# CMU-Quake/hercules

Hardware: AMD Instinct MI355X
Metric: element-updates/sec (whole node) + achieved HBM GB/s, 64M-elem box (higher is better)
Workload: dtype f64

## Files before the change

### hercules_amd/capi.py

```python
import ctypes
import os

import numpy as np

_HERE = os.path.dirname(os.path.abspath(__file__))
_LIBPATH = os.environ.get("HQ_SOLVER_LIB") or os.path.join(_HERE, "csrc", "libhq_solver.so")

HQ_VARIANT_AUTO, HQ_VARIANT_SCATTER, HQ_VARIANT_PATCH = 0, 1, 2
IPC_BLOB_BYTES = 4096

EXPORTS = ["hq_device_count", "hq_last_error", "hq_create", "hq_destroy", "hq_get_info", "hq_get_info_sized", "hq_abi_version", "hq_comm_init_ipc_n",
           "hq_options_init", "hq_create_opts", "hq_get_options", "hq_real_bytes",
           "hq_comm_unique_id", "hq_comm_init", "hq_comm_selftest", "hq_group_link", "hq_group_run", "hq_set_source", "hq_run", "hq_sync", "hq_gather", "hq_gather3",
           "hq_download", "hq_upload", "hq_phase_force", "hq_phase_update", "hq_download_force",
           "hq_run_timed", "hq_dominant_kernel", "hq_plan_check", "hq_stencil_plan_check", "hq_check_finite",
           "hq_stencil_coefficients", "hq_brick_plan_check", "hq_brick_plan_check_n", "hq_comm_init_host",
           "hq_comm_ipc_export", "hq_comm_init_ipc", "hq_comm_init_loopback"]


class HqError(RuntimeError):
    pass


HOST_EXCHANGE_FN = ctypes.CFUNCTYPE(ctypes.c_int, ctypes.c_void_p, ctypes.c_int32, ctypes.POINTER(ctypes.c_int32),
                                    ctypes.POINTER(ctypes.c_int64), ctypes.POINTER(ctypes.c_void_p), ctypes.c_int32,
                                    ctypes.POINTER(ctypes.c_int32), ctypes.POINTER(ctypes.c_int64),
                                    ctypes.POINTER(ctypes.c_void_p), ctypes.c_int32)


class _Messenger(ctypes.Structure):
    _fields_ = [("procid", ctypes.c_int32), ("nodecount", ctypes.c_int32),
                ("mapping", ctypes.c_void_p)]


class _Schedule(ctypes.Structure):
    _fields_ = [("c_count", ctypes.c_int32), ("first_c", ctypes.POINTER(_Messenger)),
                ("s_count", ctypes.c_int32), ("first_s", ctypes.POINTER(_Messenger))]


# ... 18 lines not shown
                ("ragged_patches", ctypes.c_int32), ("brick_units", ctypes.c_int32),
                ("brick_nodes", ctypes.c_int64), ("brick_units_pernode", ctypes.c_int32),
                ("brick_units_het", ctypes.c_int32), ("pcie_h2d_bytes", ctypes.c_int64),
                ("pcie_d2h_bytes", ctypes.c_int64), ("transport", ctypes.c_int32), ("ipc_arena_coarse", ctypes.c_int32),
                ("ipc_arena_kind", ctypes.c_int32), ("debug_halo", ctypes.c_int32),
                ("brick_units_packed", ctypes.c_int32), ("brick_units_ragged", ctypes.c_int32),
                ("brick_stream", ctypes.c_int32), ("brick_units_ragged_het", ctypes.c_int32), ("timed_steps", ctypes.c_int64),
                ("t_step_us", ctypes.c_double), ("t_shell_us", ctypes.c_double), ("t_interior_us", ctypes.c_double),
                ("t_chain_us", ctypes.c_double), ("t_chain_exposed_us", ctypes.c_double)]


OPTION_FIELDS = ["no_bricks", "brick_cz", "brick_minz", "brick_minnodes", "brick_no_het", "brick_no_ntsame", "brick_by_component",
                 "brick_stream", "brick_no_faces", "brick_half_tiles", "brick_no_pack", "patch_pipe", "patch_threads", "patch_pmax", "patch_pmerge", "patch_psplit", "patch_nlmax",
                 "patch_vmax", "patch_ragged", "patch_no_lattice", "patch_no_stencil", "patch_no_uniform", "patch_no_iso",
                 "patch_no_ntsame", "patch_no_dedup", "patch_wform", "patch_merge_rounds", "overlap", "no_overlap", "reserve_cus",
                 "cu_mask", "no_fused_share", "group_copies", "debug_halo", "ipc_arena"]


class Options(ctypes.Structure):
    _fields_ = ([("size", ctypes.c_uint64)] + [(n, ctypes.c_int32) for n in OPTION_FIELDS] +
                [("ipc_timeout_ms", ctypes.c_double), ("loopback_delay_us", ctypes.c_double),
                 ("verbose", ctypes.c_int32), ("quiet", ctypes.c_int32),
                 ("brick_ragged", ctypes.c_int32), ("brick_ragged_minfill", ctypes.c_int32),
                 ("allow_env", ctypes.c_int32), ("brick_ragged_het", ctypes.c_int32), ("reserved0", ctypes.c_int32),
                 ("phase_timing", ctypes.c_int32)])

    def __init__(self, **kw):
        super().__init__()
        load_library().hq_options_init(ctypes.byref(self), ctypes.c_uint64(ctypes.sizeof(self)))
        for k, v in kw.items():
            if k not in dict(self._fields_):
                raise TypeError("hq_options has no field %r" % k)
            setattr(self, k, v)

    def as_dict(self):
        return {k: getattr(self, k) for k, _ in self._fields_ if k != "size"}


_lib = None
_lib_f32 = None
_LIBPATH_F32 = os.environ.get("HQ_SOLVER_LIB_F32") or os.path.join(_HERE, "csrc", "libhq_solver_f32.so")


def load_library(path=None, precision="f64"):
    global _lib, _lib_f32
    if precision == "f32" and path is None:
        if _lib_f32 is None:
# ... 229 lines not shown
    _check(load_library().hq_plan_check(ctypes.byref(desc), rep))
    return dict(zip(PLAN_REPORT, [int(v) for v in rep]))


STENCIL_PLAN_REPORT = ("patches", "tables", "full_lattices", "boundary_nodes", "corners_checked", "faults")


def stencil_plan_check(desc):
    rep = (ctypes.c_int64 * 6)()
    _check(load_library().hq_stencil_plan_check(ctypes.byref(desc), rep))
    return dict(zip(STENCIL_PLAN_REPORT, [int(v) for v in rep]))


BRICK_PLAN_REPORT = ("brick_nodes", "columns", "units", "units_one_nt_row", "het_units", "neighbours_checked",
                     "patch_nodes", "faults", "ragged_units", "ragged_nodes", "ragged_het_units", "ragged_het_nodes")


def brick_plan_check(desc):
    rep = (ctypes.c_int64 * len(BRICK_PLAN_REPORT))()
    _check(load_library().hq_brick_plan_check_n(ctypes.byref(desc), rep, ctypes.c_int32(len(BRICK_PLAN_REPORT))))
    return dict(zip(BRICK_PLAN_REPORT, [int(v) for v in rep]))


def comm_unique_id():
    buf = (ctypes.c_char * 128)()
    _check(load_library().hq_comm_unique_id(buf))
    return bytes(buf)


def group_link(solvers):
    arr = (ctypes.c_void_p * len(solvers))(*[s._h for s in solvers])
    lib = solvers[0]._lib
    _check(lib.hq_group_link(arr, ctypes.c_int32(len(solvers))), lib)


def group_run(solvers, nsteps):
    arr = (ctypes.c_void_p * len(solvers))(*[s._h for s in solvers])
    lib = solvers[0]._lib
    _check(lib.hq_group_run(arr, ctypes.c_int32(len(solvers)), ctypes.c_int32(nsteps)), lib)
    for s in solvers:
        s.sync()
```

### hercules_amd/csrc/hq_brick.h

```cpp
#ifndef HQ_BRICK_H
#define HQ_BRICK_H

#include <chrono>
#include <map>

#include "hq_patch.h"

#define HQ_BK_TX 64
#ifndef HQ_BK_TY
#define HQ_BK_TY 8
#endif
#define HQ_BK_THREADS (HQ_BK_TX * HQ_BK_TY)
#define HQ_BK_PY (HQ_BK_TX + 2)
#define HQ_BK_PLANE ((HQ_BK_TX + 2) * (HQ_BK_TY + 2))
#ifndef HQ_BK_ATTR
#define HQ_BK_ATTR
#endif
#define HQ_BK_NTSAME 1
#define HQ_BK_HET 2
#define HQ_BK_TOPFACE 8
#define HQ_BK_BOTFACE 16
#define HQ_BK_RAGGED 32
#define HQ_BK_PACKED 4
#ifndef HQ_BH_WAVES
#define HQ_BH_WAVES 8
#endif
#define HQ_BH_THREADS (64 * HQ_BH_WAVES)
#define HQ_BH_NRT (64 + 2 * (HQ_BH_WAVES - 1))
#define HQ_BH_TX 62
#define HQ_BH_TY (HQ_BH_WAVES - 1)
#define HQ_BH_PY 65
#define HQ_BH_CS HQ_BH_THREADS
#define HQ_BH_ROWS (65 * (HQ_BH_WAVES + 1))

struct hq_brick_unit {
    int64_t base;
    int64_t tab;
    int32_t nx, ny, np, flags;
    double  c1, c2, beta;
    double  m0, m2, m1;
    double  ft[7], fb[7];
    int64_t coef;
};

struct hq_brick_cfg {
    int cz = 32;
    int minz = 4;
    int minnodes = 512;
    int ragged = 1;
    int minfill = 128;
    int ragged_het = 1;
};

static hq_brick_cfg hq_brick_cfg_of(const hq_options& o)
{
    hq_brick_cfg c;
    c.cz = std::max(2, hq_value_or(o.brick_cz, c.cz));
    c.minz = std::max(1, hq_value_or(o.brick_minz, c.minz));
    c.minnodes = std::max(1, hq_value_or(o.brick_minnodes, c.minnodes));
    c.ragged = hq_value_or(o.brick_ragged, c.ragged) != 0;
    c.minfill = std::min(HQ_BK_THREADS, std::max(1, hq_value_or(o.brick_ragged_minfill, c.minfill)));
    c.ragged_het = hq_value_or(o.brick_ragged_het, c.ragged_het) != 0;
    return c;
}

struct hq_brick_host {
// ... 672 lines not shown
        a.insert(a.end(), b.begin(), b.end());
        a.insert(a.end(), h.begin(), h.end());
        a.insert(a.end(), hp.begin(), hp.end());
        a.insert(a.end(), rh.begin(), rh.end());
        a.insert(a.end(), rhp.begin(), rhp.end());
        B->units.swap(a);
        if (B->npacked + B->nrpacked == 0) { std::vector<float>().swap(B->coef32); std::vector<double>().swap(B->nt2); }
        if (verbose) fprintf(stderr, "  brick plan: %d units: %d with one n_t row of which %d ragged, %d per-element coefficients of which %d packed, %d ragged per-element of which %d packed\n",
                             (int)B->units.size(), B->nsame, B->nrag, B->nhet, B->npacked, B->nrhet, B->nrpacked);
        if (verbose && B->nrag) {
            int64_t pos = 0, own = 0, other = 0;
            for (const hq_brick_unit& U : B->units) {
                if (!(U.flags & HQ_BK_RAGGED)) continue;
                const int32_t* pl = B->tab.data() + U.tab + (int64_t)(U.np + 2) * (2 * (U.nx + 2) + 2 * U.ny);
                for (int64_t i = 0; i < (int64_t)U.nx * U.ny * (U.np + 2); i++) { pos++; own += pl[i] >= 0; other += pl[i] <= -2; }
            }
            fprintf(stderr, "  brick plan: ragged units: %lld positions, %lld owned, %lld loaded for their neighbours' sake\n", (long long)pos, (long long)own, (long long)other);
        }
    }
    return 0;
}


static __device__ __forceinline__ double hq_uniform(double v)
{
    const int lo = __builtin_amdgcn_readfirstlane(__double2loint(v)), hi = __builtin_amdgcn_readfirstlane(__double2hiint(v));
    return __hiloint2double(hi, lo);
}

template <bool PERNODE, bool BYCOMP, bool RAGGED = false>
__global__ void HQ_BK_ATTR __launch_bounds__(HQ_BK_THREADS, 4)
hq_k_brick(int32_t count, int32_t per_xcd, const hq_brick_unit* __restrict__ units, const int32_t* __restrict__ tab,
           const hq_real* __restrict__ u1g, const hq_real* __restrict__ u2g, hq_real* __restrict__ ung,
           const double* __restrict__ nt3, const int32_t* __restrict__ src_ptr, const int32_t* __restrict__ src_ent,
           const double* __restrict__ F, double dt2, hq_stencil_coef sc)
{
    __shared__ __align__(16) double s_w[2 * 3 * HQ_BK_PLANE];
    const int slot = (int)(blockIdx.x & 7) * per_xcd + (int)(blockIdx.x >> 3);
    if (slot >= count) return;
    const hq_brick_unit U = units[slot];
    const int nx = U.nx, ny = U.ny, np = U.np, nxy = nx * ny, nr = 2 * (nx + 2) + 2 * ny;
    const int t = threadIdx.x, lx = t & (HQ_BK_TX - 1), ly = t >> 6;
    const bool active = lx < nx && ly < ny;
    const int sidx = active ? ly * nx + lx : 0;
    const int myrow = (ly + 1) * HQ_BK_PY + lx + 1;
    const bool ring = t < nr;
    int rrow;
    {
        int rx, ry;
        if (t < nx + 2) { rx = t - 1; ry = -1; }
        else if (t < 2 * (nx + 2)) { rx = t - (nx + 2) - 1; ry = ny; }
        else if (t < 2 * (nx + 2) + ny) { rx = -1; ry = t - 2 * (nx + 2); }
        else { rx = nx; ry = t - 2 * (nx + 2) - ny; }
        rrow = (ry + 1) * HQ_BK_PY + rx + 1;
    }
    const int32_t* __restrict__ utab = tab + U.tab;
    const int rofs = ring ? t : 0;
    const int32_t* __restrict__ cap = utab + (int64_t)(np + 2) * nr;
    int32_t vOut = -1, vMid = RAGGED ? cap[sidx] : 0, vCur = RAGGED ? cap[nxy + sidx] : 0, vNext = 0;
    const int32_t id_lo = RAGGED ? (vMid >= 0 ? vMid : -vMid - 2) : cap[sidx];
    const double beta = U.beta;
    double P[6], Q[2];
// ... 157 lines not shown
    }
#undef HQ_BK_LOAD
#undef HQ_BK_PUT
}


#define HQ_BH_LDS (8 * (2 * 2 * 3 * HQ_BH_ROWS + 6 * HQ_BH_THREADS))
#ifndef HQ_BH_ABL
#define HQ_BH_ABL 0
#endif

static __device__ __forceinline__ double hq_dpp_from_next_lane(double v)
{
    int lo = __double2loint(v), hi = __double2hiint(v);
    lo = __builtin_amdgcn_update_dpp(0, lo, 0x130, 0xf, 0xf, true);
    hi = __builtin_amdgcn_update_dpp(0, hi, 0x130, 0xf, 0xf, true);
    return __hiloint2double(hi, lo);
}

static __device__ __forceinline__ int64_t hq_rag_node(int32_t v) { return v >= 0 ? (int64_t)v : (v <= -2 ? (int64_t)(-v - 2) : (int64_t)0); }

template <bool PACKED, bool RAGGED = false>
__global__ void __launch_bounds__(HQ_BH_THREADS, HQ_BH_WAVES == 12 ? 3 : 4)
hq_k_brick_het(int32_t count, int32_t per_xcd, const hq_brick_unit* __restrict__ units, const int32_t* __restrict__ tab,
               const void* __restrict__ coef_any, const hq_real* __restrict__ u1g, const hq_real* __restrict__ u2g,
               hq_real* __restrict__ ung, const double* __restrict__ nt3, const int32_t* __restrict__ src_ptr,
               const int32_t* __restrict__ src_ent, const double* __restrict__ F, double dt2, hq_mat_const mat)
{
    extern __shared__ __align__(16) double s_het[];
    hq_lds_double* const img = (hq_lds_double*)s_het;
    hq_lds_double* const xch = img + 2 * 2 * 3 * HQ_BH_ROWS;
    const int slot = (int)(blockIdx.x & 7) * per_xcd + (int)(blockIdx.x >> 3);
    if (slot >= count) return;
    const hq_brick_unit U = units[slot];
    const int nx = U.nx, ny = U.ny, np = U.np, nxy = nx * ny, nr = 2 * (nx + 2) + 2 * ny;
    const int t = threadIdx.x, lx = t & 63, ly = t >> 6;
    const bool owner = lx < nx && ly < ny;
    const int sidx = owner ? ly * nx + lx : 0;
    const int myrow = (ly + 1) * HQ_BH_PY + lx + 1;
    const int row0 = ly * HQ_BH_PY + lx;
    const int rq = ly == HQ_BH_WAVES - 1 ? lx : (lx >= 62 ? 64 + 2 * ly + (lx - 62) : -1);
    const bool ringA = rq >= 0 && rq < nr, ringB = rq >= 0 && rq + HQ_BH_NRT < nr;
    auto ring_row = [&](int r) {
        int rx, ry;
        if (r < nx + 2) { rx = r - 1; ry = -1; }
        else if (r < 2 * (nx + 2)) { rx = r - (nx + 2) - 1; ry = ny; }
        else if (r < 2 * (nx + 2) + ny) { rx = -1; ry = r - 2 * (nx + 2); }
        else { rx = nx; ry = r - 2 * (nx + 2) - ny; }
        return (ry + 1) * HQ_BH_PY + rx + 1;
    };
    const int rrowA = ringA ? ring_row(rq) : 0, rrowB = ringB ? ring_row(rq + HQ_BH_NRT) : 0;
    const int32_t* __restrict__ rtabA = tab + U.tab + (ringA ? rq : 0);
    const int32_t* __restrict__ rtabB = tab + U.tab + (ringB ? rq + HQ_BH_NRT : 0);
    const int32_t* __restrict__ cap = tab + U.tab + (int64_t)(np + 2) * nr;
    const int64_t id_lo = RAGGED ? 0 : cap[sidx], id_hi = RAGGED ? 0 : cap[nxy + sidx];
    int32_t vload = RAGGED ? cap[sidx] : 0, vnext = RAGGED ? cap[nxy + sidx] : 0, idA = -1, idB = -1;
// ... 210 lines not shown
        rec.push_back({ P->h_slot[k], (int32_t)(loaded[i] - P->h_first[k]), i });
    }
    if (rec.empty()) return 0;
    std::sort(rec.begin(), rec.end());
    std::vector<int32_t> ptr((size_t)P->nunits + 1, 0), ent(rec.size() * 2);
    for (auto& r : rec) ptr[(size_t)r[0] + 1]++;
    for (int32_t u = 0; u < P->nunits; u++) ptr[(size_t)u + 1] += ptr[(size_t)u];
    for (size_t k = 0; k < rec.size(); k++) { ent[2 * k] = rec[k][1]; ent[2 * k + 1] = rec[k][2]; }
    if (hipMalloc((void**)&P->d_src_ptr, 4 * ptr.size()) != hipSuccess) { P->d_src_ptr = nullptr; return -2; }
    if (hipMalloc((void**)&P->d_src_ent, 4 * ent.size()) != hipSuccess) {
        hipFree(P->d_src_ptr); P->d_src_ptr = nullptr; P->d_src_ent = nullptr;
        return -2;
    }
    if (hipMemcpy(P->d_src_ptr, ptr.data(), 4 * ptr.size(), hipMemcpyHostToDevice) != hipSuccess ||
        hipMemcpy(P->d_src_ent, ent.data(), 4 * ent.size(), hipMemcpyHostToDevice) != hipSuccess) {
        hipFree(P->d_src_ptr); hipFree(P->d_src_ent); P->d_src_ptr = nullptr; P->d_src_ent = nullptr;
        return -3;
    }
    *bytes += (int64_t)(4 * ptr.size() + 4 * ent.size());
    return 0;
}

static void hq_brick_launch(const hq_brick_plan* P, const hq_real* u1, const hq_real* u2, hq_real* un, const double* nt3,
                            const double* F, double dt2, hipStream_t stream, bool light = false)
{
    const int32_t cnt[7] = { P->nsame - P->nrag, P->nunits - P->nsame - P->nhet - P->nrhet, P->nhet - P->npacked, P->npacked, P->nrag,
                             P->nrhet - P->nrpacked, P->nrpacked };
    int32_t first = 0;
    for (int k4 = 0; k4 < 7; k4++) {
        const int k = k4 == 0 ? 0 : (k4 == 1 ? 4 : (k4 < 5 ? k4 - 1 : k4));
        const int32_t count = cnt[k];
        if (count <= 0) continue;
        const int per_xcd = (count + 7) / 8;
        const int32_t* sp = P->d_src_ptr ? P->d_src_ptr + first : nullptr;
#define HQ_BK_ARGS count, per_xcd, P->d_units + first, P->d_tab, u1, u2, un, nt3, sp, P->d_src_ent, (sp ? F : nullptr), dt2, hq_stencil().c
#ifdef HQ_EXPERIMENT
        const unsigned xpad = getenv("HQ_X_BRICK_LDS_PAD") ? (unsigned)atoi(getenv("HQ_X_BRICK_LDS_PAD")) : 0u;
        if (xpad && k == 0) {
            static bool once = false;
            if (!once) {
                once = true;
                hipFuncSetAttribute((const void*)hq_k_brick<false, true>, hipFuncAttributeMaxDynamicSharedMemorySize, (int)xpad);
                hipFuncSetAttribute((const void*)hq_k_brick<false, false>, hipFuncAttributeMaxDynamicSharedMemorySize, (int)xpad);
            }
            if (light) hq_k_brick<false, true><<<per_xcd * 8, HQ_BK_THREADS, xpad, stream>>>(HQ_BK_ARGS);
            else hq_k_brick<false, false><<<per_xcd * 8, HQ_BK_THREADS, xpad, stream>>>(HQ_BK_ARGS);
        } else
#endif
        if (k == 0 && light) hq_k_brick<false, true><<<per_xcd * 8, HQ_BK_THREADS, 0, stream>>>(HQ_BK_ARGS);
        else if (k == 0) hq_k_brick<false, false><<<per_xcd * 8, HQ_BK_THREADS, 0, stream>>>(HQ_BK_ARGS);
        else if (k == 1 && light) hq_k_brick<true, true><<<per_xcd * 8, HQ_BK_THREADS, 0, stream>>>(HQ_BK_ARGS);
        else if (k == 1) hq_k_brick<true, false><<<per_xcd * 8, HQ_BK_THREADS, 0, stream>>>(HQ_BK_ARGS);
        else if (k == 4 && light) hq_k_brick<false, true, true><<<per_xcd * 8, HQ_BK_THREADS, 0, stream>>>(HQ_BK_ARGS);
        else if (k == 4) hq_k_brick<false, false, true><<<per_xcd * 8, HQ_BK_THREADS, 0, stream>>>(HQ_BK_ARGS);
        else if (k == 2) hq_k_brick_het<false><<<per_xcd * 8, HQ_BH_THREADS, HQ_BH_LDS, stream>>>(count, per_xcd, P->d_units + first, P->d_tab, P->d_coef, u1, u2, un, nt3, sp,
                                                                                               P->d_src_ent, (sp ? F : nullptr), dt2, P->mat);
        else if (k == 3) hq_k_brick_het<true><<<per_xcd * 8, HQ_BH_THREADS, HQ_BH_LDS, stream>>>(count, per_xcd, P->d_units + first, P->d_tab, P->d_coef32, u1, u2, un, P->d_nt2, sp,
                                                                                   P->d_src_ent, (sp ? F : nullptr), dt2, P->mat);
        else if (k == 5) hq_k_brick_het<false, true><<<per_xcd * 8, HQ_BH_THREADS, HQ_BH_LDS, stream>>>(count, per_xcd, P->d_units + first, P->d_tab, P->d_coef, u1, u2, un, nt3, sp,
                                                                                                     P->d_src_ent, (sp ? F : nullptr), dt2, P->mat);
        else hq_k_brick_het<true, true><<<per_xcd * 8, HQ_BH_THREADS, HQ_BH_LDS, stream>>>(count, per_xcd, P->d_units + first, P->d_tab, P->d_coef32, u1, u2, un, P->d_nt2, sp,
                                                                                          P->d_src_ent, (sp ? F : nullptr), dt2, P->mat);
#undef HQ_BK_ARGS
        first += count;
    }
}

#endif
```

### hercules_amd/csrc/hq_engine.hip

```cpp
#include <hip/hip_runtime.h>
#include <dlfcn.h>
#include <stdint.h>
#include <stdio.h>
#include <stdlib.h>
#include <string.h>
#include <unistd.h>

#include <algorithm>
#include <chrono>
#include <vector>

#define HQ_SOLVER_IMPLEMENTATION 1
#include "../../include/hq_solver.h"
#include "hq_kernels.h"
#include "hq_opts.h"
#include "hq_patch.h"
#include "hq_brick.h"


static thread_local char g_err[512] = "";

static int hq_fail(int code, const char* fmt, const char* a = "", const char* b = "")
{
    snprintf(g_err, sizeof g_err, fmt, a, b);
// ... 139 lines not shown
    bool overlap = false;
    bool stream_masked = false;
    bool can_overlap = false;
    int reserve_cus = 8;
    int32_t nI = 0, nOI = 0;
    double* d_iforce = nullptr;
    int32_t* d_oi_node = nullptr;
    int32_t* d_oi_slot = nullptr;
    int32_t* d_oi_ptr = nullptr;
    int32_t* d_oi_pos = nullptr;
    int32_t* d_oi_fc = nullptr;
    int32_t  nSD = 0;
    int32_t* d_sd_dst = nullptr;
    int32_t* d_sd_ptr = nullptr;
    int32_t* d_sd_src = nullptr;
    int32_t* d_sd_deps = nullptr;
    hq_patch_plan plan;
    hq_brick_plan bricks;
    std::vector<int32_t> perm;
    bool debug_halo = false;
    unsigned long long dbg_send_epoch[4] = { 0, 0, 0, 0 }, dbg_recv_epoch[4] = { 0, 0, 0, 0 };
    int64_t* d_gkey = nullptr;
    int32_t* d_halo_err = nullptr;
    enum { HQ_CLK_STEP0 = 0, HQ_CLK_SHELL1, HQ_CLK_INT0, HQ_CLK_INT1, HQ_CLK_CHAIN0, HQ_CLK_CHAIN1, HQ_CLK_N, HQ_CLK_SLOTS = 64 };
    struct hq_clock_slot { hipEvent_t e[HQ_CLK_N] = {}; bool used[HQ_CLK_N] = {}; bool pending = false; };
    bool clock_skip = false;
    std::vector<hq_clock_slot> clock;
    size_t clock_at = 0;
    double clk_us[5] = { 0, 0, 0, 0, 0 };
    int64_t clk_steps = 0;
    std::vector<hipEvent_t> ev;
    hipEvent_t ev_span[2] = { nullptr, nullptr };
    bool timing = false;
    size_t ev_used = 0;
};

template <typename T>
static int hq_dev_alloc(hq_ctx* c, T** p, size_t count)
{
    size_t bytes = sizeof(T) * (count ? count : 1);
    hipError_t e = hipMalloc((void**)p, bytes);
    if (e != hipSuccess) return hq_fail(HQ_ERR_NOMEM, "hipMalloc(%s) failed: %s", "", hipGetErrorString(e));
    c->bytes += (int64_t)bytes;
    return HQ_OK;
}

#define HQ_TRY(x) do { int r_ = (x); if (r_ != HQ_OK) return r_; } while (0)
// ... 535 lines not shown
    if (c->cstream) {
        hipError_t e2 = hipStreamSynchronize(c->cstream);
        if (e == hipSuccess) e = e2;
    }
    if (c->bstream) {
        hipError_t e2 = hipStreamSynchronize(c->bstream);
        if (e == hipSuccess) e = e2;
    }
    return e;
}

static void hq_clock_harvest(hq_ctx* c, hq_ctx::hq_clock_slot& sl, bool wait)
{
    if (!sl.pending) return;
    for (int k = 0; k < hq_ctx::HQ_CLK_N; k++)
        if (sl.used[k] && (wait ? hipEventSynchronize(sl.e[k]) : hipEventQuery(sl.e[k])) != hipSuccess) return;
    auto span = [&](int a, int b, double* us) {
        float ms = 0;
        if (!sl.used[a] || !sl.used[b] || hipEventElapsedTime(&ms, sl.e[a], sl.e[b]) != hipSuccess) return false;
        *us = 1e3 * (double)ms;
        return true;
    };
    double shell = 0, interior = 0, chain = 0, t_int_end = 0, t_chain_end = 0, t_shell_end = 0;
    span(hq_ctx::HQ_CLK_STEP0, hq_ctx::HQ_CLK_SHELL1, &shell);
    span(hq_ctx::HQ_CLK_INT0, hq_ctx::HQ_CLK_INT1, &interior);
    span(hq_ctx::HQ_CLK_CHAIN0, hq_ctx::HQ_CLK_CHAIN1, &chain);
    span(hq_ctx::HQ_CLK_STEP0, hq_ctx::HQ_CLK_SHELL1, &t_shell_end);
    span(hq_ctx::HQ_CLK_STEP0, hq_ctx::HQ_CLK_INT1, &t_int_end);
    span(hq_ctx::HQ_CLK_STEP0, hq_ctx::HQ_CLK_CHAIN1, &t_chain_end);
    const double compute_end = std::max(t_shell_end, t_int_end);
    c->clk_us[0] += std::max(compute_end, t_chain_end);
    c->clk_us[1] += shell;
    c->clk_us[2] += interior;
    c->clk_us[3] += chain;
    c->clk_us[4] += std::max(0.0, t_chain_end - compute_end);
    c->clk_steps++;
    sl.pending = false;
    for (int k = 0; k < hq_ctx::HQ_CLK_N; k++) sl.used[k] = false;
}

static void hq_clock_harvest_all(hq_ctx* c, bool wait)
{
    for (auto& sl : c->clock) hq_clock_harvest(c, sl, wait);
}

static bool hq_clock_on(const hq_ctx* c) { return hq_set(c->opts.phase_timing) || c->timing; }

// ... 149 lines not shown
        if (hipStreamCreateWithPriority(&c->bstream, hipStreamNonBlocking, prio) != hipSuccess) { c->bstream = nullptr; return false; }
        if (hipEventCreateWithFlags(&c->ev_patches, hipEventDisableTiming) != hipSuccess ||
            hipEventCreateWithFlags(&c->ev_bricks, hipEventDisableTiming) != hipSuccess) return false;
        hipEventRecord(c->ev_patches, c->stream);
        hipEventRecord(c->ev_bricks, c->stream);
    }
    return true;
}

static int hq_phase(hq_ctx* c, int ph)
{
    const bool patch = (c->variant == HQ_VARIANT_PATCH);
    double* ftab = patch ? c->d_iforce : c->d_force;
    hq_real* unew = patch ? c->d_u[c->spare] : c->d_u[c->prev];
    switch (ph) {
    case 0:
        if (patch) {
            int32_t k = c->step - c->src_step0;
            const double* F = (c->nloaded > 0 && k >= 0 && k < c->src_nsteps)
                                  ? c->d_F + (int64_t)k * c->nloaded * 3 : nullptr;
            int32_t nb = c->plan.nb, ne = c->plan.ne;
            if (c->overlap && !hq_patch_uses_pers(&c->plan) && nb > 0 && nb + ne <= 2 * hq_value_or(c->opts.patch_merge_rounds, 2) * c->plan.grid_cus) { nb += ne; ne = 0; }
            const bool bs = hq_use_brick_stream(c);
            if (c->overlap) HQ_HIP(hipStreamWaitEvent(c->stream, c->ev_shared, 0));
            if (bs) {
                HQ_HIP(hipStreamWaitEvent(c->stream, c->ev_bricks, 0));
                if (c->ev_shared) HQ_HIP(hipStreamWaitEvent(c->bstream, c->ev_shared, 0));
                HQ_HIP(hipStreamWaitEvent(c->bstream, c->ev_patches, 0));
            }
            auto launch_bricks = [&]() {
                if (c->bricks.nunits > 0)
                    hq_brick_launch(&c->bricks, c->d_u[c->now], c->d_u[c->prev], c->d_u[c->spare], c->plan.d_nt3, F, c->dt2,
                                    bs ? c->bstream : c->stream, hq_given(c->opts.brick_by_component) ? c->opts.brick_by_component != 0 : c->overlap);
                if (bs) hipEventRecord(c->ev_bricks, c->bstream);
            };
            hq_mark(c);
            hq_clock_begin(c);
            hq_clock(c, hq_ctx::HQ_CLK_STEP0, c->stream);
            if (bs) hq_clock(c, hq_ctx::HQ_CLK_INT0, c->bstream);
            bool chain_marked = false;
            auto chain_released = [&]() {
                if (!chain_marked && c->overlap) hq_clock(c, hq_ctx::HQ_CLK_CHAIN0, c->cstream);
                chain_marked = true;
            };
            if (c->plan.ns > 0 || c->plan.nr > 0) {
                const int32_t head = c->overlap ? nb : nb + ne;
                hq_patch_launch(&c->plan, 0, head, c->d_u[c->now], c->d_u[c->prev], c->d_u[c->spare], c->d_nt, F, c->dt2,
                                c->d_iforce, c->stream);
                hq_patch_launch_stencil(&c->plan, 0, c->d_u[c->now], c->d_u[c->prev], c->d_u[c->spare], c->d_nt, F, c->dt2,
                                        c->d_iforce, c->stream);
                if (c->overlap) {
                    HQ_HIP(hipEventRecord(c->ev_bnd, c->stream));
                    HQ_HIP(hipStreamWaitEvent(c->cstream, c->ev_bnd, 0));
                    chain_released();
                    hq_patch_launch(&c->plan, nb, ne, c->d_u[c->now], c->d_u[c->prev], c->d_u[c->spare], c->d_nt, F, c->dt2,
                                    c->d_iforce, c->stream, c->reserve_cus);
                }
                hq_patch_launch_stencil(&c->plan, 1, c->d_u[c->now], c->d_u[c->prev], c->d_u[c->spare], c->d_nt, F, c->dt2,
                                        c->d_iforce, c->stream);
            } else {
                if (c->overlap) {
                    hq_patch_launch(&c->plan, 0, nb, c->d_u[c->now], c->d_u[c->prev], c->d_u[c->spare], c->d_nt, F, c->dt2,
                                    c->d_iforce, c->stream);
                    HQ_HIP(hipEventRecord(c->ev_bnd, c->stream));
                    HQ_HIP(hipStreamWaitEvent(c->cstream, c->ev_bnd, 0));
                    chain_released();
                    hq_patch_launch(&c->plan, nb, ne, c->d_u[c->now], c->d_u[c->prev], c->d_u[c->spare], c->d_nt, F,
                                    c->dt2, c->d_iforce, c->stream, c->reserve_cus);
                } else {
                    hq_patch_launch(&c->plan, 0, nb + ne, c->d_u[c->now], c->d_u[c->prev], c->d_u[c->spare], c->d_nt, F,
                                    c->dt2, c->d_iforce, c->stream);
                }
            }
            if (bs) HQ_HIP(hipEventRecord(c->ev_patches, c->stream));
            hq_clock(c, hq_ctx::HQ_CLK_SHELL1, c->stream);
            if (!bs) hq_clock(c, hq_ctx::HQ_CLK_INT0, c->stream);
            launch_bricks();
            hq_clock(c, hq_ctx::HQ_CLK_INT1, bs ? c->bstream : c->stream);
            if (!c->overlap && hq_has_transport(c)) hq_clock(c, hq_ctx::HQ_CLK_CHAIN0, c->stream);
            hq_mark(c);
        } else {
            HQ_TRY(hq_launch_source(c));
            HQ_TRY(hq_launch_element_scatter(c));
        }
        return HQ_OK;
    case 1: return hq_xchg_send(c, &c->dn, ftab, true, true);
    case 2:
        HQ_TRY(hq_xchg_recv(c, &c->dn, ftab, true, true));
        if (patch) {
            if (c->nSD)
                hq_k_distribute<<<hq_blocks(c->nSD * 3, 256), 256, 0, c->overlap ? c->cstream : c->stream>>>(
                    c->nSD, c->d_sd_dst, c->d_sd_ptr, c->d_sd_src, c->d_sd_deps, c->d_iforce);
        } else if (c->nSD) {
            hq_k_distribute<<<hq_blocks(c->nSD * 3, 256), 256, 0, c->stream>>>(
                c->nSD, c->d_sd_dst, c->d_sd_ptr, c->d_sd_src, c->d_sd_deps, c->d_force);
        }
        return HQ_OK;
    case 3: return hq_xchg_send(c, &c->an, ftab, true, true);
    case 4:
        if (patch) {
            hipStream_t xs = c->overlap ? c->cstream : c->stream;
// ... 1063 lines not shown
    g_brick_check_extra[1] = 0;
    g_brick_check_extra[2] = B.nrhet;
    g_brick_check_extra[3] = 0;
    for (const hq_brick_unit& U : B.units) {
        if (!(U.flags & HQ_BK_RAGGED)) continue;
        const int32_t* pl = B.tab.data() + U.tab + (int64_t)(U.np + 2) * (2 * (U.nx + 2) + 2 * U.ny);
        for (int64_t i = (int64_t)U.nx * U.ny; i < (int64_t)U.nx * U.ny * (U.np + 1); i++) g_brick_check_extra[(U.flags & HQ_BK_HET) ? 3 : 1] += pl[i] >= 0;
    }
    if (bad) return hq_fail(HQ_ERR_STATE, "brick plan self-check failed%s", "");
    return HQ_OK;
}

extern "C" int hq_brick_plan_check_n(const hq_desc* d, int64_t* report, int32_t n)
{
    int64_t r8[8] = { 0, 0, 0, 0, 0, 0, 0, 0 };
    if (!report || n < 8) return hq_fail(HQ_ERR_ARG, "hq_brick_plan_check_n: a report of at least 8 entries%s", "");
    for (int k = 0; k < 4; k++) g_brick_check_extra[k] = 0;
    const int rc = hq_brick_plan_check(d, r8);
    for (int k = 0; k < 8; k++) report[k] = r8[k];
    for (int k = 8; k < n; k++) report[k] = k < 12 ? g_brick_check_extra[k - 8] : 0;
    return rc;
}

extern "C" int hq_destroy(hq_ctx* c)
{
    if (!c) return HQ_OK;
    hipSetDevice(c->device);
    if (c->stream) hq_quiesce(c);
    if (c->comm && g_rccl.handle) g_rccl.CommDestroy(c->comm);
    if (c->ipc) {
        hq_ipc_state* I = c->ipc;
        for (int x = 0; x < 4; x++) {
            hq_dev_schedule* sc = x < 2 ? &c->an : &c->dn;
            if (x & 1) sc->d_c_in = nullptr; else sc->d_s_in = nullptr;
            if (I->d_dst[x]) hipFree(I->d_dst[x]);
            if (I->d_sig[x]) hipFree(I->d_sig[x]);
            if (I->d_dst_id[x]) hipFree(I->d_dst_id[x]);
        }
        for (void* p : I->opened) hipIpcCloseMemHandle(p);
        if (I->d_done) hipFree(I->d_done);
        if (I->arena) hipFree(I->arena);
        delete I;
        c->ipc = nullptr;
    }
    void* ptrs[] = { c->d_gather_ids, c->d_gather_out, c->d_lnid, c->d_c1, c->d_c2, c->d_beta, c->d_nt_rows, c->d_u[0], c->d_u[1], c->d_u[2],
                     c->d_force, c->d_loaded, c->d_F, c->d_dn_id, c->d_dn_ptr, c->d_dn_anchor,
// ... 790 lines not shown
```

### hercules_amd/csrc/hq_opts.h

```cpp
#ifndef HQ_OPTS_H
#define HQ_OPTS_H

#include <cstddef>
#include <cstdlib>
#include <cstring>

struct hq_opt_entry { const char* env; size_t off; int kind; };

#define HQ_OPT_I(env_, field_) { env_, offsetof(hq_options, field_), 0 }
#define HQ_OPT_D(env_, field_) { env_, offsetof(hq_options, field_), 1 }
static const hq_opt_entry g_opt_table[] = {
    HQ_OPT_I("HQ_NO_BRICKS", no_bricks), HQ_OPT_I("HQ_BRICK_CZ", brick_cz), HQ_OPT_I("HQ_BRICK_MINZ", brick_minz),
    HQ_OPT_I("HQ_BRICK_MINNODES", brick_minnodes), HQ_OPT_I("HQ_BRICK_NO_HET", brick_no_het),
    HQ_OPT_I("HQ_BRICK_NO_NTSAME", brick_no_ntsame), HQ_OPT_I("HQ_BRICK_BY_COMPONENT", brick_by_component),
    HQ_OPT_I("HQ_BRICK_STREAM", brick_stream), HQ_OPT_I("HQ_BRICK_NO_FACES", brick_no_faces), HQ_OPT_I("HQ_BRICK_HALF_TILES", brick_half_tiles), HQ_OPT_I("HQ_BRICK_NO_PACK", brick_no_pack), HQ_OPT_I("HQ_PATCH_PIPE", patch_pipe), HQ_OPT_I("HQ_PATCH_THREADS", patch_threads),
    HQ_OPT_I("HQ_PATCH_PMAX", patch_pmax), HQ_OPT_I("HQ_PATCH_PMERGE", patch_pmerge), HQ_OPT_I("HQ_PATCH_PSPLIT", patch_psplit),
    HQ_OPT_I("HQ_PATCH_NLMAX", patch_nlmax), HQ_OPT_I("HQ_PATCH_VMAX", patch_vmax), HQ_OPT_I("HQ_PATCH_RAGGED", patch_ragged),
    HQ_OPT_I("HQ_PATCH_NO_LATTICE", patch_no_lattice), HQ_OPT_I("HQ_PATCH_NO_STENCIL", patch_no_stencil),
    HQ_OPT_I("HQ_PATCH_NO_UNIFORM", patch_no_uniform), HQ_OPT_I("HQ_PATCH_NO_ISO", patch_no_iso),
    HQ_OPT_I("HQ_PATCH_NO_NTSAME", patch_no_ntsame), HQ_OPT_I("HQ_PATCH_NO_DEDUP", patch_no_dedup),
    HQ_OPT_I("HQ_PATCH_WFORM", patch_wform), HQ_OPT_I("HQ_PATCH_MERGE_ROUNDS", patch_merge_rounds),
    HQ_OPT_I("HQ_OVERLAP", overlap), HQ_OPT_I("HQ_NO_OVERLAP", no_overlap), HQ_OPT_I("HQ_RESERVE_CUS", reserve_cus),
    HQ_OPT_I("HQ_CU_MASK", cu_mask), HQ_OPT_I("HQ_NO_FUSED_SHARE", no_fused_share), HQ_OPT_I("HQ_GROUP_COPIES", group_copies),
    HQ_OPT_I("HQ_DEBUG_HALO", debug_halo), HQ_OPT_I("HQ_IPC_ARENA", ipc_arena), HQ_OPT_D("HQ_IPC_TIMEOUT_MS", ipc_timeout_ms),
    HQ_OPT_D("HQ_LOOPBACK_DELAY_US", loopback_delay_us), HQ_OPT_I("HQ_PATCH_VERBOSE", verbose), HQ_OPT_I("HQ_QUIET", quiet),
    HQ_OPT_I("HQ_BRICK_RAGGED", brick_ragged), HQ_OPT_I("HQ_BRICK_RAGGED_MINFILL", brick_ragged_minfill),
    HQ_OPT_I("HQ_PHASE_TIMING", phase_timing), HQ_OPT_I("HQ_BRICK_RAGGED_HET", brick_ragged_het),
};
#undef HQ_OPT_I
#undef HQ_OPT_D

static void hq_options_defaults(hq_options* o)
{
    o->size = sizeof(hq_options);
    for (const hq_opt_entry& e : g_opt_table) {
        if (e.kind == 0) *(int32_t*)((char*)o + e.off) = -1;
        else *(double*)((char*)o + e.off) = -1.0;
    }
    o->allow_env = -1;
    o->reserved0 = -1;
}

static void hq_options_adopt(hq_options* dst, const hq_options* src)
{
    hq_options_defaults(dst);
    if (!src) return;
    const size_t n = (size_t)(src->size < sizeof(hq_options) ? src->size : sizeof(hq_options));
    if (n > sizeof(uint64_t)) memcpy((char*)dst + sizeof(uint64_t), (const char*)src + sizeof(uint64_t), n - sizeof(uint64_t));
    dst->size = sizeof(hq_options);
}

static int hq_opt_env_int(const char* env, const char* v)
{
    if (!strcmp(env, "HQ_IPC_ARENA")) return !strcmp(v, "fine") ? 0 : (!strcmp(v, "uncached") ? 1 : (!strcmp(v, "coarse") ? 2 : atoi(v)));
    if (!*v) return 1;
    return atoi(v);
}

static void hq_options_resolve(hq_options* out, const hq_options* caller)
{
    hq_options_adopt(out, caller);
    const char* master = getenv("HQ_ALLOW_ENV");
    const bool allow = out->allow_env >= 0 ? out->allow_env != 0 : (master && *master && strcmp(master, "0") != 0);
// ... 21 lines not shown
```

### include/hq_solver.h

```cpp
#ifndef HQ_SOLVER_H
#define HQ_SOLVER_H

#include <stdint.h>

#ifdef __cplusplus
extern "C" {
#endif

#define HQ_API __attribute__((visibility("default")))

typedef struct hq_ctx hq_ctx;

typedef enum {
    HQ_OK            =  0,
    HQ_ERR_ARG       = -1,
    HQ_ERR_NOMEM     = -2,
    HQ_ERR_DEVICE    = -3,
    HQ_ERR_NODEVICE  = -4,
    HQ_ERR_COMM      = -5,
    HQ_ERR_STATE     = -6
} hq_status;

enum {
    HQ_VARIANT_AUTO    = 0,
// ... 109 lines not shown
    int32_t patch_no_stencil;
    int32_t patch_no_uniform;
    int32_t patch_no_iso;
    int32_t patch_no_ntsame;
    int32_t patch_no_dedup;
    int32_t patch_wform;
    int32_t patch_merge_rounds;
    int32_t overlap;
    int32_t no_overlap;
    int32_t reserve_cus;
    int32_t cu_mask;
    int32_t no_fused_share;
    int32_t group_copies;
    int32_t debug_halo;
    int32_t ipc_arena;
    double  ipc_timeout_ms;
    double  loopback_delay_us;
    int32_t verbose;
    int32_t quiet;
    int32_t brick_ragged;
    int32_t brick_ragged_minfill;
    int32_t allow_env;
    int32_t brick_ragged_het;
    int32_t reserved0;
    int32_t phase_timing;
} hq_options;

HQ_API void hq_options_init(hq_options* opts, uint64_t size);
HQ_API int  hq_create_opts(const hq_desc* desc, int device, const hq_options* opts, hq_ctx** out);
HQ_API int  hq_get_options(hq_ctx* ctx, hq_options* out, uint64_t size);

HQ_API int hq_destroy(hq_ctx* ctx);

#define HQ_ABI_VERSION 6
HQ_API int hq_abi_version(void);
HQ_API int hq_real_bytes(void);
HQ_API int hq_get_info_sized(hq_ctx* ctx, hq_info* info, uint64_t size);
HQ_API int hq_get_info(hq_ctx* ctx, hq_info* info);
#ifndef HQ_SOLVER_IMPLEMENTATION
#define hq_get_info(ctx, info) hq_get_info_sized((ctx), (info), (uint64_t)sizeof(hq_info))
#endif

HQ_API int hq_comm_unique_id(void* id128);
HQ_API int hq_comm_init(hq_ctx* ctx, const void* id128);
HQ_API int hq_comm_selftest(hq_ctx* ctx, int32_t count);

typedef int (*hq_host_exchange_fn)(void* user, int32_t nrecv, const int32_t* recv_peer, const int64_t* recv_count,
// ... 18 lines not shown
HQ_API int hq_sync(hq_ctx* ctx);

HQ_API int hq_check_finite(hq_ctx* ctx, int64_t* nonfinite);

HQ_API int hq_gather(hq_ctx* ctx, int32_t n, const int32_t* lnid, hq_real* tm1_out, hq_real* tm2_out);
HQ_API int hq_gather3(hq_ctx* ctx, int32_t n, const int32_t* lnid, hq_real* tm1_out, hq_real* tm2_out,
                      hq_real* tm3_out);
HQ_API int hq_download(hq_ctx* ctx, hq_real* tm1, hq_real* tm2);
HQ_API int hq_upload(hq_ctx* ctx, const hq_real* tm1, const hq_real* tm2, int32_t step);

HQ_API int hq_phase_force(hq_ctx* ctx);
HQ_API int hq_phase_update(hq_ctx* ctx);
HQ_API int hq_download_force(hq_ctx* ctx, double* force);

HQ_API int hq_run_timed(hq_ctx* ctx, int32_t nsteps, double* total_ms, double* kernel_ms_avg);

HQ_API int hq_plan_check(const hq_desc* desc, int64_t report[8]);

HQ_API int hq_stencil_plan_check(const hq_desc* desc, int64_t report[6]);

HQ_API int hq_brick_plan_check(const hq_desc* desc, int64_t report[8]);
HQ_API int hq_brick_plan_check_n(const hq_desc* desc, int64_t* report, int32_t n);

HQ_API int hq_stencil_coefficients(double out[16]);

HQ_API const char* hq_dominant_kernel(hq_ctx* ctx);

#ifdef __cplusplus
}
#endif
#endif
```

Baseline: 61.41 billion.

## Alternate brick sweep direction and shell/interior order across steps for cache reuse

```diff
diff --git a/hercules_amd/capi.py b/hercules_amd/capi.py
--- a/hercules_amd/capi.py
+++ b/hercules_amd/capi.py
@@ -14,7 +14,7 @@
            "hq_comm_unique_id", "hq_comm_init", "hq_comm_selftest", "hq_group_link", "hq_group_run", "hq_set_source", "hq_run", "hq_sync", "hq_gather", "hq_gather3",
            "hq_download", "hq_upload", "hq_phase_force", "hq_phase_update", "hq_download_force",
            "hq_run_timed", "hq_dominant_kernel", "hq_plan_check", "hq_stencil_plan_check", "hq_check_finite",
-           "hq_stencil_coefficients", "hq_brick_plan_check", "hq_brick_plan_check_n", "hq_comm_init_host",
+           "hq_stencil_coefficients", "hq_brick_plan_check", "hq_brick_plan_check_n", "hq_brick_sweep_check", "hq_comm_init_host",
            "hq_comm_ipc_export", "hq_comm_init_ipc", "hq_comm_init_loopback"]
 
 
@@ -79,7 +79,7 @@
                 [("ipc_timeout_ms", ctypes.c_double), ("loopback_delay_us", ctypes.c_double),
                  ("verbose", ctypes.c_int32), ("quiet", ctypes.c_int32),
                  ("brick_ragged", ctypes.c_int32), ("brick_ragged_minfill", ctypes.c_int32),
-                 ("allow_env", ctypes.c_int32), ("brick_ragged_het", ctypes.c_int32), ("reserved0", ctypes.c_int32),
+                 ("allow_env", ctypes.c_int32), ("brick_ragged_het", ctypes.c_int32), ("brick_sweep", ctypes.c_int32),
                  ("phase_timing", ctypes.c_int32)])
 
     def __init__(self, **kw):
@@ -355,6 +355,18 @@
     return dict(zip(BRICK_PLAN_REPORT, [int(v) for v in rep]))
 
 
+BRICK_SWEEP_REPORT = ("workgroups", "visited", "idle", "faults")
+
+
+def brick_sweep_check(count, reverse=False):
+    grid = 8 * ((int(count) + 7) // 8)
+    slots = np.full(max(grid, 1), -2, np.int32)
+    rep = (ctypes.c_int64 * len(BRICK_SWEEP_REPORT))()
+    _check(load_library().hq_brick_sweep_check(ctypes.c_int32(count), ctypes.c_int32(1 if reverse else 0), _ptr(slots),
+                                               ctypes.c_int32(len(slots)), rep))
+    return slots[:grid], dict(zip(BRICK_SWEEP_REPORT, [int(v) for v in rep]))
+
+
 def comm_unique_id():
     buf = (ctypes.c_char * 128)()
     _check(load_library().hq_comm_unique_id(buf))
diff --git a/hercules_amd/csrc/hq_brick.h b/hercules_amd/csrc/hq_brick.h
--- a/hercules_amd/csrc/hq_brick.h
+++ b/hercules_amd/csrc/hq_brick.h
@@ -42,6 +42,10 @@
     double  ft[7], fb[7];
     int64_t coef;
 };
+
+#ifndef HQ_BRICK_SWEEP_DEFAULT
+#define HQ_BRICK_SWEEP_DEFAULT 3
+#endif
 
 struct hq_brick_cfg {
     int cz = 32;
@@ -760,6 +764,13 @@
 }
 
 
+static __host__ __device__ __forceinline__ int hq_brick_slot(int block, int per_xcd, int count, int reverse)
+{
+    const int slot = (block & 7) * per_xcd + (block >> 3);
+    if (slot >= count) return -1;
+    return reverse ? count - 1 - slot : slot;
+}
+
 static __device__ __forceinline__ double hq_uniform(double v)
 {
     const int lo = __builtin_amdgcn_readfirstlane(__double2loint(v)), hi = __builtin_amdgcn_readfirstlane(__double2hiint(v));
@@ -768,14 +779,14 @@
 
 template <bool PERNODE, bool BYCOMP, bool RAGGED = false>
 __global__ void HQ_BK_ATTR __launch_bounds__(HQ_BK_THREADS, 4)
-hq_k_brick(int32_t count, int32_t per_xcd, const hq_brick_unit* __restrict__ units, const int32_t* __restrict__ tab,
+hq_k_brick(int32_t count, int32_t per_xcd, int32_t reverse, const hq_brick_unit* __restrict__ units, const int32_t* __restrict__ tab,
            const hq_real* __restrict__ u1g, const hq_real* __restrict__ u2g, hq_real* __restrict__ ung,
            const double* __restrict__ nt3, const int32_t* __restrict__ src_ptr, const int32_t* __restrict__ src_ent,
            const double* __restrict__ F, double dt2, hq_stencil_coef sc)
 {
     __shared__ __align__(16) double s_w[2 * 3 * HQ_BK_PLANE];
-    const int slot = (int)(blockIdx.x & 7) * per_xcd + (int)(blockIdx.x >> 3);
-    if (slot >= count) return;
+    const int slot = hq_brick_slot((int)blockIdx.x, per_xcd, count, reverse);
+    if (slot < 0) return;
     const hq_brick_unit U = units[slot];
     const int nx = U.nx, ny = U.ny, np = U.np, nxy = nx * ny, nr = 2 * (nx + 2) + 2 * ny;
     const int t = threadIdx.x, lx = t & (HQ_BK_TX - 1), ly = t >> 6;
@@ -979,7 +990,7 @@
 
 template <bool PACKED, bool RAGGED = false>
 __global__ void __launch_bounds__(HQ_BH_THREADS, HQ_BH_WAVES == 12 ? 3 : 4)
-hq_k_brick_het(int32_t count, int32_t per_xcd, const hq_brick_unit* __restrict__ units, const int32_t* __restrict__ tab,
+hq_k_brick_het(int32_t count, int32_t per_xcd, int32_t reverse, const hq_brick_unit* __restrict__ units, const int32_t* __restrict__ tab,
                const void* __restrict__ coef_any, const hq_real* __restrict__ u1g, const hq_real* __restrict__ u2g,
                hq_real* __restrict__ ung, const double* __restrict__ nt3, const int32_t* __restrict__ src_ptr,
                const int32_t* __restrict__ src_ent, const double* __restrict__ F, double dt2, hq_mat_const mat)
@@ -987,8 +998,8 @@
     extern __shared__ __align__(16) double s_het[];
     hq_lds_double* const img = (hq_lds_double*)s_het;
     hq_lds_double* const xch = img + 2 * 2 * 3 * HQ_BH_ROWS;
-    const int slot = (int)(blockIdx.x & 7) * per_xcd + (int)(blockIdx.x >> 3);
-    if (slot >= count) return;
+    const int slot = hq_brick_slot((int)blockIdx.x, per_xcd, count, reverse);
+    if (slot < 0) return;
     const hq_brick_unit U = units[slot];
     const int nx = U.nx, ny = U.ny, np = U.np, nxy = nx * ny, nr = 2 * (nx + 2) + 2 * ny;
     const int t = threadIdx.x, lx = t & 63, ly = t >> 6;
@@ -1245,18 +1256,22 @@
 }
 
 static void hq_brick_launch(const hq_brick_plan* P, const hq_real* u1, const hq_real* u2, hq_real* un, const double* nt3,
-                            const double* F, double dt2, hipStream_t stream, bool light = false)
+                            const double* F, double dt2, hipStream_t stream, bool light = false, bool reverse = false)
 {
     const int32_t cnt[7] = { P->nsame - P->nrag, P->nunits - P->nsame - P->nhet - P->nrhet, P->nhet - P->npacked, P->npacked, P->nrag,
                              P->nrhet - P->nrpacked, P->nrpacked };
-    int32_t first = 0;
-    for (int k4 = 0; k4 < 7; k4++) {
-        const int k = k4 == 0 ? 0 : (k4 == 1 ? 4 : (k4 < 5 ? k4 - 1 : k4));
-        const int32_t count = cnt[k];
+    static const int order[7] = { 0, 4, 1, 2, 3, 5, 6 };
+    int32_t first_of[7];
+    for (int k4 = 0, at = 0; k4 < 7; k4++) { first_of[k4] = at; at += cnt[order[k4]] > 0 ? cnt[order[k4]] : 0; }
+    const int32_t rev = reverse ? 1 : 0;
+    for (int i4 = 0; i4 < 7; i4++) {
+        const int k4 = reverse ? 6 - i4 : i4;
+        const int k = order[k4];
+        const int32_t count = cnt[k], first = first_of[k4];
         if (count <= 0) continue;
         const int per_xcd = (count + 7) / 8;
         const int32_t* sp = P->d_src_ptr ? P->d_src_ptr + first : nullptr;
-#define HQ_BK_ARGS count, per_xcd, P->d_units + first, P->d_tab, u1, u2, un, nt3, sp, P->d_src_ent, (sp ? F : nullptr), dt2, hq_stencil().c
+#define HQ_BK_ARGS count, per_xcd, rev, P->d_units + first, P->d_tab, u1, u2, un, nt3, sp, P->d_src_ent, (sp ? F : nullptr), dt2, hq_stencil().c
 #ifdef HQ_EXPERIMENT
         const unsigned xpad = getenv("HQ_X_BRICK_LDS_PAD") ? (unsigned)atoi(getenv("HQ_X_BRICK_LDS_PAD")) : 0u;
         if (xpad && k == 0) {
@@ -1276,16 +1291,15 @@
         else if (k == 1) hq_k_brick<true, false><<<per_xcd * 8, HQ_BK_THREADS, 0, stream>>>(HQ_BK_ARGS);
         else if (k == 4 && light) hq_k_brick<false, true, true><<<per_xcd * 8, HQ_BK_THREADS, 0, stream>>>(HQ_BK_ARGS);
         else if (k == 4) hq_k_brick<false, false, true><<<per_xcd * 8, HQ_BK_THREADS, 0, stream>>>(HQ_BK_ARGS);
-        else if (k == 2) hq_k_brick_het<false><<<per_xcd * 8, HQ_BH_THREADS, HQ_BH_LDS, stream>>>(count, per_xcd, P->d_units + first, P->d_tab, P->d_coef, u1, u2, un, nt3, sp,
+        else if (k == 2) hq_k_brick_het<false><<<per_xcd * 8, HQ_BH_THREADS, HQ_BH_LDS, stream>>>(count, per_xcd, rev, P->d_units + first, P->d_tab, P->d_coef, u1, u2, un, nt3, sp,
                                                                                                P->d_src_ent, (sp ? F : nullptr), dt2, P->mat);
-        else if (k == 3) hq_k_brick_het<true><<<per_xcd * 8, HQ_BH_THREADS, HQ_BH_LDS, stream>>>(count, per_xcd, P->d_units + first, P->d_tab, P->d_coef32, u1, u2, un, P->d_nt2, sp,
+        else if (k == 3) hq_k_brick_het<true><<<per_xcd * 8, HQ_BH_THREADS, HQ_BH_LDS, stream>>>(count, per_xcd, rev, P->d_units + first, P->d_tab, P->d_coef32, u1, u2, un, P->d_nt2, sp,
                                                                                    P->d_src_ent, (sp ? F : nullptr), dt2, P->mat);
-        else if (k == 5) hq_k_brick_het<false, true><<<per_xcd * 8, HQ_BH_THREADS, HQ_BH_LDS, stream>>>(count, per_xcd, P->d_units + first, P->d_tab, P->d_coef, u1, u2, un, nt3, sp,
+        else if (k == 5) hq_k_brick_het<false, true><<<per_xcd * 8, HQ_BH_THREADS, HQ_BH_LDS, stream>>>(count, per_xcd, rev, P->d_units + first, P->d_tab, P->d_coef, u1, u2, un, nt3, sp,
                                                                                                      P->d_src_ent, (sp ? F : nullptr), dt2, P->mat);
-        else hq_k_brick_het<true, true><<<per_xcd * 8, HQ_BH_THREADS, HQ_BH_LDS, stream>>>(count, per_xcd, P->d_units + first, P->d_tab, P->d_coef32, u1, u2, un, P->d_nt2, sp,
+        else hq_k_brick_het<true, true><<<per_xcd * 8, HQ_BH_THREADS, HQ_BH_LDS, stream>>>(count, per_xcd, rev, P->d_units + first, P->d_tab, P->d_coef32, u1, u2, un, P->d_nt2, sp,
                                                                                           P->d_src_ent, (sp ? F : nullptr), dt2, P->mat);
 #undef HQ_BK_ARGS
-        first += count;
     }
 }
 
diff --git a/hercules_amd/csrc/hq_engine.hip b/hercules_amd/csrc/hq_engine.hip
--- a/hercules_amd/csrc/hq_engine.hip
+++ b/hercules_amd/csrc/hq_engine.hip
@@ -185,7 +185,7 @@
     unsigned long long dbg_send_epoch[4] = { 0, 0, 0, 0 }, dbg_recv_epoch[4] = { 0, 0, 0, 0 };
     int64_t* d_gkey = nullptr;
     int32_t* d_halo_err = nullptr;
-    enum { HQ_CLK_STEP0 = 0, HQ_CLK_SHELL1, HQ_CLK_INT0, HQ_CLK_INT1, HQ_CLK_CHAIN0, HQ_CLK_CHAIN1, HQ_CLK_N, HQ_CLK_SLOTS = 64 };
+    enum { HQ_CLK_STEP0 = 0, HQ_CLK_SHELL1, HQ_CLK_INT0, HQ_CLK_INT1, HQ_CLK_CHAIN0, HQ_CLK_CHAIN1, HQ_CLK_SHELL0, HQ_CLK_N, HQ_CLK_SLOTS = 64 };
     struct hq_clock_slot { hipEvent_t e[HQ_CLK_N] = {}; bool used[HQ_CLK_N] = {}; bool pending = false; };
     bool clock_skip = false;
     std::vector<hq_clock_slot> clock;
@@ -767,7 +767,7 @@
         return true;
     };
     double shell = 0, interior = 0, chain = 0, t_int_end = 0, t_chain_end = 0, t_shell_end = 0;
-    span(hq_ctx::HQ_CLK_STEP0, hq_ctx::HQ_CLK_SHELL1, &shell);
+    span(sl.used[hq_ctx::HQ_CLK_SHELL0] ? hq_ctx::HQ_CLK_SHELL0 : hq_ctx::HQ_CLK_STEP0, hq_ctx::HQ_CLK_SHELL1, &shell);
     span(hq_ctx::HQ_CLK_INT0, hq_ctx::HQ_CLK_INT1, &interior);
     span(hq_ctx::HQ_CLK_CHAIN0, hq_ctx::HQ_CLK_CHAIN1, &chain);
     span(hq_ctx::HQ_CLK_STEP0, hq_ctx::HQ_CLK_SHELL1, &t_shell_end);
@@ -963,6 +963,11 @@
             int32_t nb = c->plan.nb, ne = c->plan.ne;
             if (c->overlap && !hq_patch_uses_pers(&c->plan) && nb > 0 && nb + ne <= 2 * hq_value_or(c->opts.patch_merge_rounds, 2) * c->plan.grid_cus) { nb += ne; ne = 0; }
             const bool bs = hq_use_brick_stream(c);
+            const int sweep = hq_value_or(c->opts.brick_sweep, (int32_t)HQ_BRICK_SWEEP_DEFAULT);
+            const bool odd = (c->step & 1) != 0;
+            const bool sweep_rev = (sweep & 1) && odd;
+            const bool shell_last = (sweep & 2) && !odd && !bs && !c->overlap && !hq_has_transport(c) && c->nranks == 1 &&
+                                    c->ldnnum == 0 && c->nSD == 0 && c->nOI == 0 && c->bricks.nunits > 0 && c->plan.npatches > 0;
             if (c->overlap) HQ_HIP(hipStreamWaitEvent(c->stream, c->ev_shared, 0));
             if (bs) {
                 HQ_HIP(hipStreamWaitEvent(c->stream, c->ev_bricks, 0));
@@ -972,13 +977,20 @@
             auto launch_bricks = [&]() {
                 if (c->bricks.nunits > 0)
                     hq_brick_launch(&c->bricks, c->d_u[c->now], c->d_u[c->prev], c->d_u[c->spare], c->plan.d_nt3, F, c->dt2,
-                                    bs ? c->bstream : c->stream, hq_given(c->opts.brick_by_component) ? c->opts.brick_by_component != 0 : c->overlap);
+                                    bs ? c->bstream : c->stream, hq_given(c->opts.brick_by_component) ? c->opts.brick_by_component != 0 : c->overlap,
+                                    sweep_rev);
                 if (bs) hipEventRecord(c->ev_bricks, c->bstream);
             };
             hq_mark(c);
             hq_clock_begin(c);
             hq_clock(c, hq_ctx::HQ_CLK_STEP0, c->stream);
             if (bs) hq_clock(c, hq_ctx::HQ_CLK_INT0, c->bstream);
+            if (shell_last) {
+                hq_clock(c, hq_ctx::HQ_CLK_INT0, c->stream);
+                launch_bricks();
+                hq_clock(c, hq_ctx::HQ_CLK_INT1, c->stream);
+                hq_clock(c, hq_ctx::HQ_CLK_SHELL0, c->stream);
+            }
             bool chain_marked = false;
             auto chain_released = [&]() {
                 if (!chain_marked && c->overlap) hq_clock(c, hq_ctx::HQ_CLK_CHAIN0, c->cstream);
@@ -1015,9 +1027,11 @@
             }
             if (bs) HQ_HIP(hipEventRecord(c->ev_patches, c->stream));
             hq_clock(c, hq_ctx::HQ_CLK_SHELL1, c->stream);
-            if (!bs) hq_clock(c, hq_ctx::HQ_CLK_INT0, c->stream);
-            launch_bricks();
-            hq_clock(c, hq_ctx::HQ_CLK_INT1, bs ? c->bstream : c->stream);
+            if (!shell_last) {
+                if (!bs) hq_clock(c, hq_ctx::HQ_CLK_INT0, c->stream);
+                launch_bricks();
+                hq_clock(c, hq_ctx::HQ_CLK_INT1, bs ? c->bstream : c->stream);
+            }
             if (!c->overlap && hq_has_transport(c)) hq_clock(c, hq_ctx::HQ_CLK_CHAIN0, c->stream);
             hq_mark(c);
         } else {
@@ -2127,6 +2141,30 @@
     return rc;
 }
 
+extern "C" int hq_brick_sweep_check(int32_t count, int32_t reverse, int32_t* slot_of_block, int32_t n, int64_t report[4])
+{
+    if (count < 0 || !report) return hq_fail(HQ_ERR_ARG, "hq_brick_sweep_check: bad argument%s", "");
+    const int per_xcd = (count + 7) / 8, grid = 8 * per_xcd;
+    if (slot_of_block && n < grid) return hq_fail(HQ_ERR_ARG, "hq_brick_sweep_check: room for 8 * ceil(count / 8) workgroups%s", "");
+    std::vector<int32_t> seen((size_t)count, 0);
+    int64_t visited = 0, faults = 0, idle = 0;
+    int last[8];
+    for (int x = 0; x < 8; x++) last[x] = -1;
+    for (int b = 0; b < grid; b++) {
+        const int slot = hq_brick_slot(b, per_xcd, count, reverse);
+        if (slot_of_block) slot_of_block[b] = slot;
+        if (slot < 0) { idle++; continue; }
+        if (slot >= count || seen[(size_t)slot]++) { faults++; continue; }
+        visited++;
+        int& l = last[b & 7];
+        if (l >= 0 && slot != (reverse ? l - 1 : l + 1)) faults++;
+        l = slot;
+    }
+    if (visited != count) faults++;
+    report[0] = grid; report[1] = visited; report[2] = idle; report[3] = faults;
+    return HQ_OK;
+}
+
 extern "C" int hq_destroy(hq_ctx* c)
 {
     if (!c) return HQ_OK;
diff --git a/hercules_amd/csrc/hq_opts.h b/hercules_amd/csrc/hq_opts.h
--- a/hercules_amd/csrc/hq_opts.h
+++ b/hercules_amd/csrc/hq_opts.h
@@ -26,6 +26,7 @@
     HQ_OPT_D("HQ_LOOPBACK_DELAY_US", loopback_delay_us), HQ_OPT_I("HQ_PATCH_VERBOSE", verbose), HQ_OPT_I("HQ_QUIET", quiet),
     HQ_OPT_I("HQ_BRICK_RAGGED", brick_ragged), HQ_OPT_I("HQ_BRICK_RAGGED_MINFILL", brick_ragged_minfill),
     HQ_OPT_I("HQ_PHASE_TIMING", phase_timing), HQ_OPT_I("HQ_BRICK_RAGGED_HET", brick_ragged_het),
+    HQ_OPT_I("HQ_BRICK_SWEEP", brick_sweep),
 };
 #undef HQ_OPT_I
 #undef HQ_OPT_D
@@ -38,7 +39,6 @@
         else *(double*)((char*)o + e.off) = -1.0;
     }
     o->allow_env = -1;
-    o->reserved0 = -1;
 }
 
 static void hq_options_adopt(hq_options* dst, const hq_options* src)
diff --git a/include/hq_solver.h b/include/hq_solver.h
--- a/include/hq_solver.h
+++ b/include/hq_solver.h
@@ -155,7 +155,7 @@
     int32_t brick_ragged_minfill;
     int32_t allow_env;
     int32_t brick_ragged_het;
-    int32_t reserved0;
+    int32_t brick_sweep;
     int32_t phase_timing;
 } hq_options;
 
@@ -220,6 +220,8 @@
 HQ_API int hq_brick_plan_check(const hq_desc* desc, int64_t report[8]);
 HQ_API int hq_brick_plan_check_n(const hq_desc* desc, int64_t* report, int32_t n);
 
+HQ_API int hq_brick_sweep_check(int32_t count, int32_t reverse, int32_t* slot_of_block, int32_t n, int64_t report[4]);
+
 HQ_API int hq_stencil_coefficients(double out[16]);
 
 HQ_API const char* hq_dominant_kernel(hq_ctx* ctx);
```

Result: no change. 61.13 billion (-0.5%).
